# joaobuibergen/roms-trunk-mgh

Hardware: AMD Instinct MI355X
Metric: simulated-days/wall-sec (higher is better)
Workload: dtype f64; 1 GPU; BENCHMARK3 2048x256x30 NT=2 nonlinear 3-D step incl. 59 step2d calls, U3/C4 tracer advection, analytic atmospheric forcing, bulk fluxes + KPP + diagnostics every step; tiling=1x1, halo_transport=none, rccl_ranks=0, graph_exchanges=1, ndtfast=20, finite=True

## Files before the change

roms_trunk_mgh_amd/csrc/advect.h:

```cpp
#pragma once
#include <type_traits>
#include "roms_dev.h"

template <int HADV>
__device__ __forceinline__ double hflux(double Hflx, double tm1, double t0, double dm1, double d0, double dp1)
{
  if constexpr (HADV == ADV_C2) {
    return Hflx * 0.5 * (tm1 + t0);
  } else if constexpr (HADV == ADV_MPDATA) {
    const double cff1 = fmax(Hflx, 0.0), cff2 = fmin(Hflx, 0.0);
    return cff1 * tm1 + cff2 * t0;
  } else if constexpr (HADV == ADV_U3) {
    const double curv_m1 = d0 - dm1;
    const double curv_0 = dp1 - d0;
    const double cff1 = 1.0 / 6.0;
    return Hflx * 0.5 * (tm1 + t0) -
           cff1 * (curv_m1 * fmax(Hflx, 0.0) + curv_0 * fmin(Hflx, 0.0));
  } else if constexpr (HADV == ADV_A4) {
    const double eps = 1.0E-16;
    double g_m1, g_0;
    double cff = 2.0 * d0 * dm1;
    g_m1 = (cff > eps) ? cff / (d0 + dm1) : 0.0;
    cff = 2.0 * dp1 * d0;
    g_0 = (cff > eps) ? cff / (dp1 + d0) : 0.0;
// ... 147 lines not shown
  f.FEjp1 = hflux<HADV>(s.hv1, tk, s.yp1, dy0, dyp1, dyp2);
  return f;
}
template <int VADV>
__device__ __forceinline__ double vflux_level(int k, int N, double Wk, double tkm1, double tk, double tkp1, double tkp2,
                                              const double *spl, const double *a4cf)
{
  if (k == N) return 0.0;
  if constexpr (VADV == ADV_SPLINES) return spl[k];
  else {
    double cfk = 0.0, cfk1 = 0.0;
    if constexpr (VADV == ADV_A4) { cfk = a4cf[k]; cfk1 = a4cf[k + 1]; }
    return vflux<VADV>(k, N, Wk, tkm1, tk, tkp1, tkp2, cfk, cfk1);
  }
}
__device__ __forceinline__ void thomas_row(double dt, double hz_m1, double ohz_m1, double hz, double ohz, double akt_m2,
                                           double akt_m1, double akt_0, double t_m1, double t_0, double CFm, double DCm,
                                           double &CF, double &DC)
{
  const double cff6 = 1.0 / 6.0, cff3r = 1.0 / 3.0;
  const double fc = cff6 * hz_m1 - dt * akt_m2 * ohz_m1;
  const double cf = cff6 * hz - dt * akt_0 * ohz;
  const double bc = cff3r * (hz_m1 + hz) + dt * akt_m1 * (ohz_m1 + ohz);
  const double cff = 1.0 / (bc - fc * CFm);
  CF = cff * cf;
  DC = cff * (t_0 - t_m1 - fc * DCm);
}

static inline int adv_pair(int ha, int va)
{
// ... 25 lines not shown
```

roms_trunk_mgh_amd/csrc/k_mix.hip:

```cpp
#include "roms_dev.h"

int roms_entry_check(const char *name);

namespace {

__device__ __forceinline__ double dmin0(double a) { return a < 0.0 ? a : 0.0; }
__device__ __forceinline__ double dmax0(double a) { return a > 0.0 ? a : 0.0; }

template <bool STAB>
__device__ __forceinline__ double tdiff(double a, double b, double a2, double b2)
{
  if constexpr (STAB) return 0.75 * (a - b) + 0.25 * (a2 - b2);
  else return a - b;
}

struct Lap4 {
  double *lap;
  int i0, i1, j0, j1;
  int closed[4];
  int itrc;
  int nstp;
};

template <int MODE>
__device__ __forceinline__ void lap4_store(const roms_bounds_t &b, const Lap4 &L, long ni, int i, int j, long a, double val)
{
  const gd_t lap = (gd_t)L.lap;
  lap[a] = val;
  if (!b.EWperiodic) {
    if (b.west_edge && i == b.Istr) lap[a - 1] = L.closed[LBS_WEST] ? 0.0 : val;
    if (b.east_edge && i == b.Iend) lap[a + 1] = L.closed[LBS_EAST] ? 0.0 : val;
  }
  if (!b.NSperiodic) {
    if (b.south_edge && j == b.Jstr) lap[a - ni] = L.closed[LBS_SOUTH] ? 0.0 : val;
    if (b.north_edge && j == b.Jend) lap[a + ni] = L.closed[LBS_NORTH] ? 0.0 : val;
  }
}

template <int MODE, bool ISO, bool STAB = false>
__global__ void __launch_bounds__(BLK_X *BLK_Y)
k_t3dmix_geo(const RomsDev *__restrict__ c, int nrhs, int nnew, Lap4 L)
{
  DEV_PROLOGUE(c)
  const int ilo = MODE == 1 ? L.i0 : b.Istr, ihi = MODE == 1 ? L.i1 : b.Iend;
  const int jlo = MODE == 1 ? L.j0 : b.Jstr, jhi = MODE == 1 ? L.j1 : b.Jend;
  const TileTr tt = decode_tile_tracer(ihi - ilo + 1, jhi - jlo + 1, MODE == 0 ? b.NT : 1);
  if (!tt.valid) return;
  const int i = ilo + tt.bx * BLK_X + threadIdx.x;
  const int j = jlo + tt.by * BLK_Y + threadIdx.y;
  const int itrc = MODE == 0 ? 1 + tt.itr : L.itrc;
  if (i > ihi || j > jhi) return;
  const double dt = c->p.dt;
  const double *__restrict__ T = MODE == 2 ? L.lap : c->F.t + ((long)(nrhs - 1) + 3L * (itrc - 1)) * n3r;
  static_assert(!(STAB && MODE == 2), "the second biharmonic operator acts on LapT alone");
  const double *__restrict__ S = STAB ? c->F.t + ((long)(L.nstp - 1) + 3L * (itrc - 1)) * n3r : T;
  double *__restrict__ tn = c->F.t + ((long)(nnew - 1) + 3L * (itrc - 1)) * n3r;
  const double *__restrict__ z_r = ISO ? c->F.pden : c->F.z_r;
// ... 16 lines not shown
    mx0 = mx0 * umaskw(c, c0); mx1 = mx1 * umaskw(c, c0 + 1);
    my0 = my0 * vmaskw(c, c0); my1 = my1 * vmaskw(c, c0 + ni);
  }
  const double cfx0 = 0.25 * (d2[c0] + d2[c0 - 1]) * c->F.on_u[c0];
  const double cfx1 = 0.25 * (d2[c0 + 1] + d2[c0]) * c->F.on_u[c0 + 1];
  const double cfe0 = 0.25 * (d2[c0] + d2[c0 - ni]) * c->F.om_v[c0];
  const double cfe1 = 0.25 * (d2[c0 + ni] + d2[c0]) * c->F.om_v[c0 + ni];
  const double cfs = 0.5 * d2[c0];
  const double cdt = dt * pm[c0] * pn[c0];
  double zx0_a, zx1_a, tx0_a, tx1_a, ze0_a, ze1_a, te0_a, te1_a;
  double zx0_b, zx1_b, tx0_b, tx1_b, ze0_b, ze1_b, te0_b, te1_b;
  double dzm_a = 0.0, dz0_a = 0.0, dzp_a = 0.0, dzs_a = 0.0, dzn_a = 0.0;
  double dzm_b, dz0_b, dzp_b, dzs_b, dzn_b;
  double FS_a = 0.0, FS_b;
  double fsf_b = 0.0;
  struct LvIn { double Tm1, T01, Tp1, Ts1, Tn1, Zm1, Z01, Zp1, Zs1, Zn1, hz0, hzm, hzp, hzs, hzn, tn, zz1;
                double Sm1, S01, Sp1, Ss1, Sn1;
                double zzm1, zzp1, zzs1, zzn1; };
  const gcd_t gT = (gcd_t)T, gS = (gcd_t)S, gZ = (gcd_t)z_r, gHz = (gcd_t)Hz;
  const gd_t gtn = (gd_t)tn;
  auto load_level = [&](int k) {
    LvIn L;
    const long ck = c0 + (long)(k - 1) * nij;
    const long cu = (k < N) ? ck + nij : ck;
    L.Tm1 = gT[cu - 1]; L.T01 = gT[cu]; L.Tp1 = gT[cu + 1]; L.Ts1 = gT[cu - ni]; L.Tn1 = gT[cu + ni];
    if constexpr (STAB) { L.Sm1 = gS[cu - 1]; L.S01 = gS[cu]; L.Sp1 = gS[cu + 1]; L.Ss1 = gS[cu - ni]; L.Sn1 = gS[cu + ni]; }
    else L.Sm1 = L.S01 = L.Sp1 = L.Ss1 = L.Sn1 = 0.0;
    L.Zm1 = gZ[cu - 1]; L.Z01 = gZ[cu]; L.Zp1 = gZ[cu + 1]; L.Zs1 = gZ[cu - ni]; L.Zn1 = gZ[cu + ni];
    L.hz0 = gHz[ck]; L.hzm = gHz[ck - 1]; L.hzp = gHz[ck + 1]; L.hzs = gHz[ck - ni]; L.hzn = gHz[ck + ni];
    L.tn = gtn[ck];
    if constexpr (ISO) L.zz1 = ((gcd_t)zz)[cu]; else L.zz1 = 0.0;
    L.zzm1 = L.zzp1 = L.zzs1 = L.zzn1 = 0.0;
    if (minstrat) {
      const gcd_t gz = (gcd_t)zz;
      L.zzm1 = gz[cu - 1]; L.zzp1 = gz[cu + 1]; L.zzs1 = gz[cu - ni]; L.zzn1 = gz[cu + ni];
    }
    return L;
  };
  double Tm = T[c0 - 1], T0 = T[c0], Tp = T[c0 + 1], Ts = T[c0 - ni], Tn = T[c0 + ni];
  double Sm = 0.0, S0 = 0.0, Sp = 0.0, Ss = 0.0, Sn = 0.0;
  if constexpr (STAB) { Sm = S[c0 - 1]; S0 = S[c0]; Sp = S[c0 + 1]; Ss = S[c0 - ni]; Sn = S[c0 + ni]; }
  double Zm = z_r[c0 - 1], Z0 = z_r[c0], Zp = z_r[c0 + 1], Zs = z_r[c0 - ni], Zn = z_r[c0 + ni];
  double zzc = ISO ? zz[c0] : 0.0;
  double zzm = 0.0, zzp = 0.0, zzs = 0.0, zzn = 0.0;
  if (minstrat) { zzm = zz[c0 - 1]; zzp = zz[c0 + 1]; zzs = zz[c0 - ni]; zzn = zz[c0 + ni]; }
  zx0_b = mx0 * (Z0 - Zm); tx0_b = mx0 * tdiff<STAB>(T0, Tm, S0, Sm);
  zx1_b = mx1 * (Zp - Z0); tx1_b = mx1 * tdiff<STAB>(Tp, T0, Sp, S0);
  ze0_b = my0 * (Z0 - Zs); te0_b = my0 * tdiff<STAB>(T0, Ts, S0, Ss);
  ze1_b = my1 * (Zn - Z0); te1_b = my1 * tdiff<STAB>(Tn, T0, Sn, S0);
  LvIn cur = load_level(1);
  for (int k = 1; k <= N; k++) {
    const long ck = c0 + (long)(k - 1) * nij;
    LvIn nxt = cur;
    if (k < N) nxt = load_level(k + 1);
    zx0_a = zx0_b; zx1_a = zx1_b; tx0_a = tx0_b; tx1_a = tx1_b;
    ze0_a = ze0_b; ze1_a = ze1_b; te0_a = te0_b; te1_a = te1_b;
    if (k < N) {
      const double Tm1 = cur.Tm1, T01 = cur.T01, Tp1 = cur.Tp1, Ts1 = cur.Ts1, Tn1 = cur.Tn1;
      const double Zm1 = cur.Zm1, Z01 = cur.Z01, Zp1 = cur.Zp1, Zs1 = cur.Zs1, Zn1 = cur.Zn1;
      const double Sm1 = cur.Sm1, S01 = cur.S01, Sp1 = cur.Sp1, Ss1 = cur.Ss1, Sn1 = cur.Sn1;
      zx0_b = mx0 * (Z01 - Zm1); tx0_b = mx0 * tdiff<STAB>(T01, Tm1, S01, Sm1);
      zx1_b = mx1 * (Zp1 - Z01); tx1_b = mx1 * tdiff<STAB>(Tp1, T01, Sp1, S01);
      ze0_b = my0 * (Z01 - Zs1); te0_b = my0 * tdiff<STAB>(T01, Ts1, S01, Ss1);
      ze1_b = my1 * (Zn1 - Z01); te1_b = my1 * tdiff<STAB>(Tn1, T01, Sn1, S01);
      { const double q = vscale(Zm, Zm1, cur.zzm1 - zzm); dzm_b = q * tdiff<STAB>(Tm1, Tm, Sm1, Sm); }
      { const double q = vscale(Z0, Z01, cur.zz1 - zzc); dz0_b = q * tdiff<STAB>(T01, T0, S01, S0);
        if constexpr (ISO) { fsf_b = q * (cur.zz1 - zzc); zzc = cur.zz1; } }
// ... 37 lines not shown
        c1 = f1(ze0_a); c2 = f1(ze1_b); c3 = f2(ze0_b); c4 = f2(ze1_a);
        cff = cff + cfs * (c1 * (c1 * dz0_b - te0_a) + c2 * (c2 * dz0_b - te1_b) +
                           c3 * (c3 * dz0_b - te0_b) + c4 * (c4 * dz0_b - te1_a));
        FS_b = cff * fsf_b;
      }
    } else FS_b = 0.0;
    if constexpr (MODE == 1) {
      const double cff = pm[c0] * pn[c0];
      const double cff1 = 1.0 / hz0;
      lap4_store<MODE>(b, L, ni, i, j, ck, cff1 * (cff * (FX1 - FX0 + FE1 - FE0) + (FS_b - FS_a)));
    } else {
      const double cff1 = cdt * (FX1 - FX0);
      const double cff2 = cdt * (FE1 - FE0);
      const double cff3 = dt * (FS_b - FS_a);
      const double cff4 = cff1 + cff2 + cff3;
      if constexpr (MODE == 0) gtn[ck] = cur.tn + cff4;
      else gtn[ck] = cur.tn - cff4;
    }
    cur = nxt;
    dzm_a = dzm_b; dz0_a = dz0_b; dzp_a = dzp_b; dzs_a = dzs_b; dzn_a = dzn_b;
    FS_a = FS_b;
  }
}

template <bool STAB, bool DIA = false>
__global__ void __launch_bounds__(BLK_X *BLK_Y)
k_t3dmix2_s(const RomsDev *__restrict__ c, int nrhs, int nnew, int nstp)
{
  DEV_PROLOGUE(c)
  const TileTr tt = decode_tile_tracer(b.Iend - b.Istr + 1, b.Jend - b.Jstr + 1, b.NT);
  if (!tt.valid) return;
// ... 80 lines not shown
    double FE1 = cfe1 * (Hz[ck + ni] + h0) * tdiff<STAB>(T[ck + ni], t0, sn, s0);
    if constexpr (MODE == 1) {
      const double cff = 1.0 / h0;
      lap4_store<MODE>(b, L, ni, i, j, ck, pmn * cff * (FX1 - FX0 + FE1 - FE0));
    } else {
      if (masking) { FX0 = FX0 * um0; FX1 = FX1 * um1; FE0 = FE0 * vm0; FE1 = FE1 * vm1; }
      const double cff1 = cdt * (FX1 - FX0);
      const double cff2 = cdt * (FE1 - FE0);
      tn[ck] = tn[ck] - (cff1 + cff2);
    }
  }
}

}

static int t3dmix2_launch(const roms_step_idx_t *s)
{
  const roms_bounds_t &b = g_ctx.b;
  const dim3 grid = grid_tile_tracer(b.Iend - b.Istr + 1, b.Jend - b.Jstr + 1, b.NT);
  const bool stab = g_ctx.p.ts_mix_stability != 0;
  Lap4 L{};
  L.nstp = s->nstp;
  if (g_ctx.p.mix_iso_ts) {
    if (stab) hipLaunchKernelGGL((k_t3dmix_geo<0, true, true>), grid, block2d(), 0, g_ctx.stream, g_ctx.devc, s->nrhs, s->nnew, L);
    else hipLaunchKernelGGL((k_t3dmix_geo<0, true>), grid, block2d(), 0, g_ctx.stream, g_ctx.devc, s->nrhs, s->nnew, L);
  } else if (g_ctx.p.mix_geo_ts) {
    if (stab) hipLaunchKernelGGL((k_t3dmix_geo<0, false, true>), grid, block2d(), 0, g_ctx.stream, g_ctx.devc, s->nrhs, s->nnew, L);
    else hipLaunchKernelGGL((k_t3dmix_geo<0, false>), grid, block2d(), 0, g_ctx.stream, g_ctx.devc, s->nrhs, s->nnew, L);
  } else if (g_ctx.p.mix_s_ts && dia_on()) {
    if (stab) hipLaunchKernelGGL((k_t3dmix2_s<true, true>), grid, block2d(), 0, g_ctx.stream, g_ctx.devc, s->nrhs, s->nnew, s->nstp);
    else hipLaunchKernelGGL((k_t3dmix2_s<false, true>), grid, block2d(), 0, g_ctx.stream, g_ctx.devc, s->nrhs, s->nnew, s->nstp);
  } else if (g_ctx.p.mix_s_ts) {
    if (stab) hipLaunchKernelGGL(k_t3dmix2_s<true>, grid, block2d(), 0, g_ctx.stream, g_ctx.devc, s->nrhs, s->nnew, s->nstp);
    else hipLaunchKernelGGL(k_t3dmix2_s<false>, grid, block2d(), 0, g_ctx.stream, g_ctx.devc, s->nrhs, s->nnew, s->nstp);
  } else
    return roms_fail("roms_hip_t3dmix2", "no tracer mixing option (MIX_ISO_TS / MIX_GEO_TS / MIX_S_TS) selected");
  KERNEL_CHECK("k_t3dmix2");
  return 0;
}

extern "C" int roms_hip_t3dmix2(const roms_step_idx_t *s)
{
  int rc = roms_entry_check("roms_hip_t3dmix2");
  if (rc) return rc;
  if ((rc = dia_check("roms_hip_t3dmix2"))) return rc;
  if (dia_on() && !g_ctx.p.ts_dif2)
    return roms_fail("roms_hip_t3dmix2", "diagnostics: ts_dif2 is off, the iT?dif terms have no planes (NDT = 6)");
  ScopedTimer tm("t3dmix2");
  return t3dmix2_launch(s);
}

extern "C" int roms_hip_t3dmix4(const roms_step_idx_t *s)
{
  int rc = roms_entry_check("roms_hip_t3dmix4");
  if (rc) return rc;
  const roms_bounds_t &b = g_ctx.b;
  const roms_params_t &p = g_ctx.p;
  if (!p.ts_dif4) return roms_fail("roms_hip_t3dmix4", "TS_DIF4 is not set (roms_params_t.ts_dif4)");
  if ((rc = dia_check("roms_hip_t3dmix4"))) return rc;
  if (!p.mix_iso_ts && !p.mix_geo_ts && !p.mix_s_ts)
    return roms_fail("roms_hip_t3dmix4", "no tracer mixing option (MIX_ISO_TS / MIX_GEO_TS / MIX_S_TS) selected");
  ScopedTimer tm("t3dmix4");
  const bool stab = p.ts_mix_stability != 0;
  Lap4 L;
  L.lap = g_ctx.hostc.ws3[1];
// ... 28 lines not shown
```

roms_trunk_mgh_amd/csrc/k_pre_step3d.hip:

```cpp
#include "roms_dev.h"
#include "advect.h"

int roms_entry_check(const char *name);

namespace {

template <int HADV, int VADV, int NMAX, bool MASK, bool DIA = false>
__global__ void __launch_bounds__(BLK_X *BLK_Y)
k_pre_t(const RomsDev *__restrict__ c, int nstp, int nnew, int first_step, int itrc0, int ntr)
{
  DEV_PROLOGUE(c)
  const TileCol tc = tile_column(b, itrc0, ntr);
  if (!tc.valid) return;
  const int i = tc.i, j = tc.j, itrc = tc.itrc;
  const roms_params_t &p = c->p;
  const double dt = p.dt;
  const gcd_t ts = (gcd_t)tracer_level(c, nstp, itrc, n3r);
  const gd_t t3 = (gd_t)tracer_level(c, 3, itrc, n3r);
  const gd_t tn = (gd_t)tracer_level(c, nnew, itrc, n3r);
  const ColFields f = column_fields(c);
  const gcd_t z_r = (gcd_t)(c->F.z_r);
  const gcd_t z_w = (gcd_t)(c->F.z_w);
  const gcd_t Akt = tracer_akt(c, itrc, n3w);
  const long c0 = I2(i, j);
  const Walls wl = column_walls(c, i, j);
  const double Gamma = (HADV == ADV_MPDATA) ? 0.5 : 1.0 / 6.0;
  const double GammaV = (VADV == ADV_MPDATA) ? 0.5 : 1.0 / 6.0;
  double cff, cff1, cff2;
  if (first_step) { cff = 0.5 * dt; cff1 = 1.0; cff2 = 0.0; }
  else { cff = (1.0 - Gamma) * dt; cff1 = 0.5 + Gamma; cff2 = 0.5 - Gamma; }
  const double cpp = cff * GF(pm)[c0] * GF(pn)[c0];
  const double cppv = (first_step ? 0.5 * dt : (1.0 - GammaV) * dt) * GF(pm)[c0] * GF(pn)[c0];
  const double cff3 = dt * (1.0 - p.lambda);
  const bool nonlocal = p.lmd_nonlocal && itrc <= b.NAT;
  const bool solar = p.solar_source && itrc == 1;
  const gcd_t ghats = (gcd_t)(c->F.ghats + (long)((itrc <= b.NAT ? itrc : 1) - 1) * n3w);
  const gcd_t AktN = (gcd_t)(c->F.Akt + (long)((itrc <= b.NAT ? itrc : 1) - 1) * n3w);
  const double srf = GF(srflx)[c0];
  const double dsrf = c->p.wet_dry ? (dt * srf) * GF(rmask_wet)[c0] : dt * srf;
  const double zwN = z_w[c0 + (long)N * nij];
  const double fac1 = -1.0 / p.swfrac_mu1, fac2 = -1.0 / p.swfrac_mu2, fac3 = p.swfrac_r1;

  double a4cf[(VADV == ADV_A4) ? NMAX + 2 : 1];
  double spl[(VADV == ADV_SPLINES) ? NMAX + 1 : 1];
  if constexpr (VADV == ADV_A4) a4_slopes<NMAX>(ts, c0, nij, N, a4cf);
  if constexpr (VADV == ADV_SPLINES) spline_w<true, NMAX>(ts, f.Hz, f.W, c0, nij, N, spl);

  const bool src_cell = c->src.n > 0 && src_cell_any(c, c0, ni);
  double tkm1 = 0.0, tk = ts[c0], tkp1 = (N >= 2) ? ts[c0 + nij] : 0.0, tkp2;
  double FCprev = 0.0;
  double FDprev = dt * GF(btflx)[c0 + (long)(itrc - 1) * nij];
  double w_km1 = f.W[c0];
  double zr_k = (cff3 != 0.0) ? z_r[c0] : 0.0;
  for (int k = 1; k <= N; k++) {
    const long ck = c0 + (long)(k - 1) * nij;
    tkp2 = (k + 2 <= N) ? ts[ck + 2 * nij] : 0.0;
    HStencil s;
    s.xm1 = ts[ck - 1]; s.xp1 = ts[ck + 1];
    s.xm2 = wl.w ? 0.0 : ts[ck - 2];
    s.xp2 = wl.e ? 0.0 : ts[ck + 2];
    s.ym1 = ts[ck - ni]; s.yp1 = ts[ck + ni];
    s.ym2 = wl.s ? 0.0 : ts[ck - 2 * ni];
    s.yp2 = wl.n ? 0.0 : ts[ck + 2 * ni];
    s.hu0 = f.Huon[ck]; s.hu1 = f.Huon[ck + 1];
    s.hv0 = f.Hvom[ck]; s.hv1 = f.Hvom[ck + ni];
    Faces fx = cell_faces<HADV, MASK>(tk, s, wl, c, c0, ni);
    if (src_cell)
      src_cell_fluxes<true>(c, c0, ck, ni, k, itrc, nullptr, fx.FXi, fx.FXip1, fx.FEj, fx.FEjp1);
    const double hz = f.Hz[ck];
    const double tnn = tn[ck];
    double t3v = hz * (cff1 * tk + cff2 * tnn) - cpp * (fx.FXip1 - fx.FXi + fx.FEjp1 - fx.FEj);
    const double w_k = f.W[ck + nij];
    const double FCk = vflux_level<VADV>(k, N, w_k, tkm1, tk, tkp1, tkp2, spl, a4cf);
    const double DCk = 1.0 / (hz - cppv * (s.hu1 - s.hu0 + s.hv1 - s.hv0 + (w_k - w_km1)));
    t3v = DCk * (t3v - cppv * (FCk - FCprev));
    t3[ck] = t3v;
    double FDk;
    if (k == N) FDk = dt * GF(stflx)[c0 + (long)(itrc - 1) * nij];
    else {
      if (cff3 != 0.0) {
        const double zr_k1 = z_r[ck + nij];
        const double cz = 1.0 / (zr_k1 - zr_k);
        FDk = cff3 * cz * Akt[ck + nij] * (tkp1 - tk);
        zr_k = zr_k1;
      } else {
        FDk = 0.0;
      }
      if (nonlocal) FDk = FDk - dt * AktN[ck + nij] * ghats[ck + nij];
      if (solar) {
        const double Z = zwN - z_w[ck + nij];
        const double swdk = exp(Z * fac1) * fac3 + exp(Z * fac2) * (1.0 - fac3);
        FDk = FDk + dsrf * swdk;
      }
    }
    const double hzt = hz * tk, dFD = FDk - FDprev;
    tn[ck] = hzt + dFD;
    if constexpr (DIA) {
      DIA_PLANE(c, DIA_iTrate, itrc, n3r)[ck] = hzt;
      DIA_PLANE(c, DIA_iTvdif, itrc, n3r)[ck] = dFD;
    }
    FDprev = FDk;
    FCprev = FCk;
    w_km1 = w_k;
    tkm1 = tk; tk = tkp1; tkp1 = tkp2;
  }
}

__global__ void __launch_bounds__(BLK_X *BLK_Y)
k_pre_uv(const RomsDev *__restrict__ c, int nstp, int nnew, int nrhs, int stage)
{
  DEV_PROLOGUE(c)
  const Blk XB = xcd_block();
  const int i = b.Istr + XB.x * BLK_X + threadIdx.x;
  const int j = b.Jstr + XB.y * BLK_Y + threadIdx.y;
  if (i > b.Iend || j > b.Jend) return;
  const roms_params_t &p = c->p;
  const double dt = p.dt;
  const double cff3 = dt * (1.0 - p.lambda);
  const gcd_t z_r = (gcd_t)(c->F.z_r);
// ... 42 lines not shown
      } else if (stage == 1) {
        const double a = vk * 0.5 * hzs;
        const double c3 = 0.5 * DC0;
        out = a - c3 * r2[ck + nij] + d;
      } else {
        const double a = vk * 0.5 * hzs;
        out = a + DC0 * ((5.0 / 12.0) * r1[ck + nij] - (16.0 / 12.0) * r2[ck + nij]) + d;
      }
      vnew[ck] = out;
      FCprev = FCk;
      vk = vk1;
    }
  }
}

template <int HADV, int VADV>
int launch_pre_t(const roms_step_idx_t *s, int itrc0, int ntr)
{
  typedef void (*PreKernel)(const RomsDev *, int, int, int, int, int);
  const roms_bounds_t &b = g_ctx.b;
  const dim3 grid = grid_tile_tracer(b.Iend - b.Istr + 1, b.Jend - b.Jstr + 1, ntr);
  const int first = s->iic == s->ntfirst;
  if (b.N > ROMS_MAXN) return roms_fail("roms_hip_pre_step3d", "N > 64 not instantiated");
  PreKernel kernel = kernel_for_n(b.N, [](auto nm) -> PreKernel { return k_pre_t<HADV, VADV, nm.value, false>; });
  if constexpr (HADV != ADV_MPDATA)
    if (g_ctx.p.masking)
      kernel = kernel_for_n(b.N, [](auto nm) -> PreKernel { return k_pre_t<HADV, VADV, nm.value, true>; });
  if constexpr (HADV != ADV_MPDATA && VADV != ADV_MPDATA)
    if (dia_on())
      kernel = g_ctx.p.masking ? k_pre_t<HADV, VADV, ROMS_MAXN, true, true> : k_pre_t<HADV, VADV, ROMS_MAXN, false, true>;
  hipLaunchKernelGGL(kernel, grid, block2d(), 0, g_ctx.stream, g_ctx.devc, s->nstp, s->nnew, first, itrc0, ntr);
  KERNEL_CHECK("k_pre_t");
  return 0;
}

}

static int pre_step3d_tracers(const roms_step_idx_t *s)
{
  const roms_bounds_t &b = g_ctx.b;
  const roms_params_t &p = g_ctx.p;
  int rc = 0;
  {
    int it = 1;
    while (it <= b.NT) {
      const int n = adv_run_length(p, b.NT, it);
      switch (adv_pair(p.Hadv[it - 1], p.Vadv[it - 1])) {
      case ADV_U3 * 16 + ADV_C4:   rc = launch_pre_t<ADV_U3, ADV_C4>(s, it, n); break;
      case ADV_A4 * 16 + ADV_A4:   rc = launch_pre_t<ADV_A4, ADV_A4>(s, it, n); break;
      case ADV_C4 * 16 + ADV_C4:   rc = launch_pre_t<ADV_C4, ADV_C4>(s, it, n); break;
      case ADV_C2 * 16 + ADV_C2:   rc = launch_pre_t<ADV_C2, ADV_C2>(s, it, n); break;
      case ADV_U3 * 16 + ADV_SPLINES: rc = launch_pre_t<ADV_U3, ADV_SPLINES>(s, it, n); break;
      case ADV_C4 * 16 + ADV_SPLINES: rc = launch_pre_t<ADV_C4, ADV_SPLINES>(s, it, n); break;
      case ADV_A4 * 16 + ADV_SPLINES: rc = launch_pre_t<ADV_A4, ADV_SPLINES>(s, it, n); break;
      case ADV_MPDATA * 16 + ADV_MPDATA: rc = launch_pre_t<ADV_MPDATA, ADV_MPDATA>(s, it, n); break;
      case ADV_HSIMT * 16 + ADV_HSIMT: rc = launch_pre_t<ADV_MPDATA, ADV_MPDATA>(s, it, n); break;
      case ADV_U3 * 16 + ADV_HSIMT: rc = launch_pre_t<ADV_U3, ADV_MPDATA>(s, it, n); break;
      case ADV_C4 * 16 + ADV_HSIMT: rc = launch_pre_t<ADV_C4, ADV_MPDATA>(s, it, n); break;
      case ADV_A4 * 16 + ADV_HSIMT: rc = launch_pre_t<ADV_A4, ADV_MPDATA>(s, it, n); break;
      case ADV_C2 * 16 + ADV_HSIMT: rc = launch_pre_t<ADV_C2, ADV_MPDATA>(s, it, n); break;
      default:
        return roms_fail("roms_hip_pre_step3d", "advection scheme pair not implemented (MPDATA and HSIMT only as H+V pairs)");
      }
      if (rc) return rc;
      it += n;
    }
  }
  const long n3r = (long)(b.UBi - b.LBi + 1) * (b.UBj - b.LBj + 1) * b.N;
  for (int it = 1; it <= b.NT; it++)
    if ((rc = bc_t3d(3, it, s->nstp))) return rc;
  halo_batch_begin();
  for (int it = 1; it <= b.NT; it++) halo_exchange3d(GT_R, b.N, g_ctx.dev[FID_t] + (2L + 3L * (it - 1)) * n3r);
  return halo_batch_end();
}

static int pre_step3d_uv(const roms_step_idx_t *s)
{
  const roms_bounds_t &b = g_ctx.b;
  const int stage = (s->iic == s->ntfirst) ? 0 : (s->iic == s->ntfirst + 1 ? 1 : 2);
  hipLaunchKernelGGL(k_pre_uv, grid2d(b.Iend - b.Istr + 1, b.Jend - b.Jstr + 1), block2d(), 0, g_ctx.stream,
                     g_ctx.devc, s->nstp, s->nnew, s->nrhs, stage);
  KERNEL_CHECK("k_pre_uv");
  return 0;
}

extern "C" int roms_hip_pre_step3d(const roms_step_idx_t *s)
{
  int rc = roms_entry_check("roms_hip_pre_step3d");
  if (rc) return rc;
  if ((rc = check_lbc())) return rc;
  if (g_ctx.b.N < 4) return roms_fail("roms_hip_pre_step3d", "needs N >= 4 levels (the vertical stencils of the column read k-1 .. k+2)");
  if ((rc = dia_check("roms_hip_pre_step3d"))) return rc;
  ScopedTimer tm("pre_step3d");
  if ((rc = pre_step3d_uv(s))) return rc;
  return pre_step3d_tracers(s);
}
```

roms_trunk_mgh_amd/csrc/k_rhs3d.hip:

```cpp
#include "roms_dev.h"

namespace {

#define Gadv (-0.25)

struct T3 {
  const double *u, *v, *Hu, *Hv, *Hz;
  int i0, j0;
  int Istr, Iend, Jstr, Jend;
  bool s_edge, n_edge, w_edge, e_edge;
  __device__ __forceinline__ int at(int i, int j) const { return (i - i0) + (j - j0) * TP; }
};

__device__ __forceinline__ int ex_uxx(const T3 &L, int i) {
  if (L.w_edge && i == L.Istr) return L.Istr + 1;
  if (L.e_edge && i == L.Iend + 1) return L.Iend;
  return i;
}
__device__ __forceinline__ int ey_uee(const T3 &L, int j) {
  if (L.s_edge && j == L.Jstr - 1) return L.Jstr;
  if (L.n_edge && j == L.Jend + 1) return L.Jend;
  return j;
}
__device__ __forceinline__ int ex_vxx(const T3 &L, int i) {
// ... 391 lines not shown
                                            : (spl ? k_rhs3d_lds<ROMS_UVH_U3, ROMS_UVV_SPLINES> : k_rhs3d_lds<ROMS_UVH_U3, ROMS_UVV_C4W>);
  hipLaunchKernelGGL(kernel, grid2d(b.Iend - b.Istr + 1, b.Jend - b.Jstr + 1), block2d(), 0, g_ctx.stream,
                     g_ctx.devc, s->nrhs);
  KERNEL_CHECK("k_rhs3d_lds");
  if (spl) {
    const dim3 grid((unsigned)((b.Iend - b.Istr + BLK_X) / BLK_X), (unsigned)(b.Jend - b.Jstr + 1), 1), block(BLK_X, 1, 1);
    if (b.N <= 16) hipLaunchKernelGGL(k_rhs3d_vspline<16>, grid, block, 0, g_ctx.stream, g_ctx.devc, s->nrhs);
    else if (b.N <= 32) hipLaunchKernelGGL(k_rhs3d_vspline<32>, grid, block, 0, g_ctx.stream, g_ctx.devc, s->nrhs);
    else if (b.N <= 48) hipLaunchKernelGGL(k_rhs3d_vspline<48>, grid, block, 0, g_ctx.stream, g_ctx.devc, s->nrhs);
    else hipLaunchKernelGGL(k_rhs3d_vspline<64>, grid, block, 0, g_ctx.stream, g_ctx.devc, s->nrhs);
    KERNEL_CHECK("k_rhs3d_vspline");
  }
  return 0;
}

extern "C" int roms_hip_rhs3d(const roms_step_idx_t *s)
{
  int rc = roms_entry_check("roms_hip_rhs3d");
  if (rc) return rc;
  if ((rc = roms_uv_adv_check("roms_hip_rhs3d"))) return rc;
  if ((rc = roms_hip_pre_step3d(s))) return rc;
  if ((rc = roms_hip_prsgrd(s))) return rc;
  if (g_ctx.p.ts_dif2 && (rc = roms_hip_t3dmix2(s))) return rc;
  if (g_ctx.p.ts_dif4 && (rc = roms_hip_t3dmix4(s))) return rc;
  if ((rc = roms_hip_rhs3d_tile(s))) return rc;
  if (g_ctx.p.uv_vis2 && (rc = roms_hip_uv3dmix2(s))) return rc;
  if (g_ctx.p.uv_vis4 && (rc = roms_hip_uv3dmix4(s))) return rc;
  return 0;
}
```

roms_trunk_mgh_amd/csrc/roms_dev.h:

```cpp
#pragma once
#include <hip/hip_runtime.h>
#include <cstdio>
#include <cstring>
#include <string>
#include "roms_hip.h"

#define ROMS_NWS3 10

struct RomsSrc {
  int n;
  int ltr[ROMS_MAXNT];
  const int *I, *J, *D;
  const double *Qbar;
  const double *Qsrc;
  const double *Tsrc;
  const int *umap, *vmap;
  const int *wmap;
  const int *cells;
  int ncell;
  double *save;
};

struct RomsClima {
  int m2, m3, nt;
// ... 295 lines not shown
int dia_arrays(const char *name[4], const double *base[4], long count[4]);
int bc_zeta(int kout, const roms_step_idx_t *s);
int bc_u2d(int kout, const roms_step_idx_t *s);
int bc_v2d(int kout, const roms_step_idx_t *s);
int bc_u3d(int nout, int nstp);
int bc_v3d(int nout, int nstp);
int bc_t3d(int nout, int itrc, int nstp);
bool lbc2d_all_closed();
int lbc_code(const roms_params_t &p, int sd, int v);
int bc_w3d(double *A);
int bc_generic(int gtype_var, int lbv, double *A, int nk);
void snapshot_release();
void snapshot_forget(int field_id);
void diag_release();
int check_lbc();
int roms_rowm_prepare();
void roms_rowm_invalidate();
bool roms_rowm_is_table_field(int id);
void roms_rowm_release();
void step2d_graphs_release();
```

Baseline: 0.2365 simulated-days/s.

## Defer tracer t(nnew) start into t3dmix2 and pair tracers in pre_step3d

When harmonic geopotential or isopycnal tracer mixing runs with lambda=1, no stability mixing and no diagnostics, pre_step3d no longer writes t(nnew). It writes only t(3). The Hz*t plus vertical-flux start of t(nnew) is computed inside the t3dmix2 kernel, which already writes that plane, so one read-modify-write pass over t(nnew) is removed. The deferred pre_t kernel also processes two tracers per thread, sharing the Huon, Hvom, Hz and W loads and the DCk divide. In exchange it uses more registers and adds template instantiations, and it only applies under restrictive runtime conditions.

```diff
diff --git a/roms_trunk_mgh_amd/csrc/advect.h b/roms_trunk_mgh_amd/csrc/advect.h
--- a/roms_trunk_mgh_amd/csrc/advect.h
+++ b/roms_trunk_mgh_amd/csrc/advect.h
@@ -185,6 +185,68 @@
     return vflux<VADV>(k, N, Wk, tkm1, tk, tkp1, tkp2, cfk, cfk1);
   }
 }
+struct VStart {
+  double dt, cff3, dsrf, zwN, fac1, fac2, fac3;
+  bool nonlocal, solar;
+  gcd_t Akt, AktN, ghats, z_r, z_w;
+  int itrc;
+};
+__device__ __forceinline__ VStart vstart_column(const RomsDev *__restrict__ c, int itrc, long c0, long nij, long n3w)
+{
+  const roms_params_t &p = c->p;
+  const roms_bounds_t &b = c->b;
+  VStart v;
+  v.dt = p.dt;
+  v.cff3 = p.dt * (1.0 - p.lambda);
+  v.nonlocal = p.lmd_nonlocal && itrc <= b.NAT;
+  v.solar = p.solar_source && itrc == 1;
+  v.Akt = tracer_akt(c, itrc, n3w);
+  v.ghats = (gcd_t)(c->F.ghats + (long)((itrc <= b.NAT ? itrc : 1) - 1) * n3w);
+  v.AktN = (gcd_t)(c->F.Akt + (long)((itrc <= b.NAT ? itrc : 1) - 1) * n3w);
+  v.z_r = (gcd_t)(c->F.z_r);
+  v.z_w = (gcd_t)(c->F.z_w);
+  const double srf = GF(srflx)[c0];
+  v.dsrf = p.wet_dry ? (p.dt * srf) * GF(rmask_wet)[c0] : p.dt * srf;
+  v.zwN = v.z_w[c0 + (long)b.N * nij];
+  v.fac1 = -1.0 / p.swfrac_mu1; v.fac2 = -1.0 / p.swfrac_mu2; v.fac3 = p.swfrac_r1;
+  v.itrc = itrc;
+  return v;
+}
+struct VStartIn { double akn, gh, zwk; };
+__device__ __forceinline__ VStartIn vstart_load(const VStart &v, long cku)
+{
+  VStartIn r{0.0, 0.0, 0.0};
+  if (v.nonlocal) { r.akn = v.AktN[cku]; r.gh = v.ghats[cku]; }
+  if (v.solar) r.zwk = v.z_w[cku];
+  return r;
+}
+__device__ __forceinline__ double vstart_bottom(const RomsDev *__restrict__ c, const VStart &v, long c0, long nij)
+{
+  return v.dt * GF(btflx)[c0 + (long)(v.itrc - 1) * nij];
+}
+template <bool EXPL>
+__device__ __forceinline__ double vstart_flux(const RomsDev *__restrict__ c, const VStart &v, int k, int N, long c0, long nij,
+                                              long cku, const VStartIn &in, double tk, double tkp1, double &zr_k)
+{
+  if (k == N) return v.dt * GF(stflx)[c0 + (long)(v.itrc - 1) * nij];
+  double FDk = 0.0;
+  if constexpr (EXPL) {
+    if (v.cff3 != 0.0) {
+      const double zr_k1 = v.z_r[cku];
+      const double cz = 1.0 / (zr_k1 - zr_k);
+      FDk = v.cff3 * cz * v.Akt[cku] * (tkp1 - tk);
+      zr_k = zr_k1;
+    }
+  }
+  if (v.nonlocal) FDk = FDk - v.dt * in.akn * in.gh;
+  if (v.solar) {
+    const double Z = v.zwN - in.zwk;
+    const double swdk = exp(Z * v.fac1) * v.fac3 + exp(Z * v.fac2) * (1.0 - v.fac3);
+    FDk = FDk + v.dsrf * swdk;
+  }
+  return FDk;
+}
+
 __device__ __forceinline__ void thomas_row(double dt, double hz_m1, double ohz_m1, double hz, double ohz, double akt_m2,
                                            double akt_m1, double akt_0, double t_m1, double t_0, double CFm, double DCm,
                                            double &CF, double &DC)
diff --git a/roms_trunk_mgh_amd/csrc/k_mix.hip b/roms_trunk_mgh_amd/csrc/k_mix.hip
--- a/roms_trunk_mgh_amd/csrc/k_mix.hip
+++ b/roms_trunk_mgh_amd/csrc/k_mix.hip
@@ -1,4 +1,5 @@
 #include "roms_dev.h"
+#include "advect.h"
 
 int roms_entry_check(const char *name);
 
@@ -37,10 +38,11 @@
   }
 }
 
-template <int MODE, bool ISO, bool STAB = false>
+template <int MODE, bool ISO, bool STAB = false, bool START = false>
 __global__ void __launch_bounds__(BLK_X *BLK_Y)
 k_t3dmix_geo(const RomsDev *__restrict__ c, int nrhs, int nnew, Lap4 L)
 {
+  static_assert(!START || (MODE == 0 && !STAB), "the corrector's start goes with t3dmix2 alone");
   DEV_PROLOGUE(c)
   const int ilo = MODE == 1 ? L.i0 : b.Istr, ihi = MODE == 1 ? L.i1 : b.Iend;
   const int jlo = MODE == 1 ? L.j0 : b.Jstr, jhi = MODE == 1 ? L.j1 : b.Jend;
@@ -87,9 +89,13 @@
   double dzm_b, dz0_b, dzp_b, dzs_b, dzn_b;
   double FS_a = 0.0, FS_b;
   double fsf_b = 0.0;
+  VStart vs{};
+  double FDprev = 0.0, zr_unused = 0.0;
+  if constexpr (START) { vs = vstart_column(c, itrc, c0, nij, n3w); FDprev = vstart_bottom(c, vs, c0, nij); }
   struct LvIn { double Tm1, T01, Tp1, Ts1, Tn1, Zm1, Z01, Zp1, Zs1, Zn1, hz0, hzm, hzp, hzs, hzn, tn, zz1;
                 double Sm1, S01, Sp1, Ss1, Sn1;
-                double zzm1, zzp1, zzs1, zzn1; };
+                double zzm1, zzp1, zzs1, zzn1;
+                double akn, gh, zwk; };
   const gcd_t gT = (gcd_t)T, gS = (gcd_t)S, gZ = (gcd_t)z_r, gHz = (gcd_t)Hz;
   const gd_t gtn = (gd_t)tn;
   auto load_level = [&](int k) {
@@ -101,7 +107,10 @@
     else L.Sm1 = L.S01 = L.Sp1 = L.Ss1 = L.Sn1 = 0.0;
     L.Zm1 = gZ[cu - 1]; L.Z01 = gZ[cu]; L.Zp1 = gZ[cu + 1]; L.Zs1 = gZ[cu - ni]; L.Zn1 = gZ[cu + ni];
     L.hz0 = gHz[ck]; L.hzm = gHz[ck - 1]; L.hzp = gHz[ck + 1]; L.hzs = gHz[ck - ni]; L.hzn = gHz[ck + ni];
-    L.tn = gtn[ck];
+    if constexpr (START) L.tn = 0.0; else L.tn = gtn[ck];
+    L.akn = L.gh = L.zwk = 0.0;
+    if constexpr (START)
+      if (k < N) { const VStartIn in = vstart_load(vs, ck + nij); L.akn = in.akn; L.gh = in.gh; L.zwk = in.zwk; }
     if constexpr (ISO) L.zz1 = ((gcd_t)zz)[cu]; else L.zz1 = 0.0;
     L.zzm1 = L.zzp1 = L.zzs1 = L.zzn1 = 0.0;
     if (minstrat) {
@@ -124,6 +133,7 @@
   LvIn cur = load_level(1);
   for (int k = 1; k <= N; k++) {
     const long ck = c0 + (long)(k - 1) * nij;
+    const double Tk = T0;
     LvIn nxt = cur;
     if (k < N) nxt = load_level(k + 1);
     zx0_a = zx0_b; zx1_a = zx1_b; tx0_a = tx0_b; tx1_a = tx1_b;
@@ -191,7 +201,13 @@
       const double cff2 = cdt * (FE1 - FE0);
       const double cff3 = dt * (FS_b - FS_a);
       const double cff4 = cff1 + cff2 + cff3;
-      if constexpr (MODE == 0) gtn[ck] = cur.tn + cff4;
+      if constexpr (START) {
+        const VStartIn in{cur.akn, cur.gh, cur.zwk};
+        const double FDk = vstart_flux<false>(c, vs, k, N, c0, nij, ck + nij, in, Tk, 0.0, zr_unused);
+        const double hzt = hz0 * Tk, dFD = FDk - FDprev;
+        gtn[ck] = (hzt + dFD) + cff4;
+        FDprev = FDk;
+      } else if constexpr (MODE == 0) gtn[ck] = cur.tn + cff4;
       else gtn[ck] = cur.tn - cff4;
     }
     cur = nxt;
@@ -302,14 +318,19 @@
 
 }
 
-static int t3dmix2_launch(const roms_step_idx_t *s)
+static int t3dmix2_launch(const roms_step_idx_t *s, bool fused)
 {
   const roms_bounds_t &b = g_ctx.b;
   const dim3 grid = grid_tile_tracer(b.Iend - b.Istr + 1, b.Jend - b.Jstr + 1, b.NT);
   const bool stab = g_ctx.p.ts_mix_stability != 0;
   Lap4 L{};
   L.nstp = s->nstp;
-  if (g_ctx.p.mix_iso_ts) {
+  if (fused) {
+    if (stab || dia_on() || !(g_ctx.p.mix_iso_ts || g_ctx.p.mix_geo_ts))
+      return roms_fail("roms_hip_t3dmix2", "internal: the fused start of t(nnew) was asked for where it is not built");
+    if (g_ctx.p.mix_iso_ts) hipLaunchKernelGGL((k_t3dmix_geo<0, true, false, true>), grid, block2d(), 0, g_ctx.stream, g_ctx.devc, s->nrhs, s->nnew, L);
+    else hipLaunchKernelGGL((k_t3dmix_geo<0, false, false, true>), grid, block2d(), 0, g_ctx.stream, g_ctx.devc, s->nrhs, s->nnew, L);
+  } else if (g_ctx.p.mix_iso_ts) {
     if (stab) hipLaunchKernelGGL((k_t3dmix_geo<0, true, true>), grid, block2d(), 0, g_ctx.stream, g_ctx.devc, s->nrhs, s->nnew, L);
     else hipLaunchKernelGGL((k_t3dmix_geo<0, true>), grid, block2d(), 0, g_ctx.stream, g_ctx.devc, s->nrhs, s->nnew, L);
   } else if (g_ctx.p.mix_geo_ts) {
@@ -327,7 +348,7 @@
   return 0;
 }
 
-extern "C" int roms_hip_t3dmix2(const roms_step_idx_t *s)
+int t3dmix2_entry(const roms_step_idx_t *s, bool fused)
 {
   int rc = roms_entry_check("roms_hip_t3dmix2");
   if (rc) return rc;
@@ -335,8 +356,10 @@
   if (dia_on() && !g_ctx.p.ts_dif2)
     return roms_fail("roms_hip_t3dmix2", "diagnostics: ts_dif2 is off, the iT?dif terms have no planes (NDT = 6)");
   ScopedTimer tm("t3dmix2");
-  return t3dmix2_launch(s);
-}
+  return t3dmix2_launch(s, fused);
+}
+
+extern "C" int roms_hip_t3dmix2(const roms_step_idx_t *s) { return t3dmix2_entry(s, false); }
 
 extern "C" int roms_hip_t3dmix4(const roms_step_idx_t *s)
 {
diff --git a/roms_trunk_mgh_amd/csrc/k_pre_step3d.hip b/roms_trunk_mgh_amd/csrc/k_pre_step3d.hip
--- a/roms_trunk_mgh_amd/csrc/k_pre_step3d.hip
+++ b/roms_trunk_mgh_amd/csrc/k_pre_step3d.hip
@@ -5,23 +5,20 @@
 
 namespace {
 
-template <int HADV, int VADV, int NMAX, bool MASK, bool DIA = false>
+template <int HADV, int VADV, int NMAX, bool MASK, bool DIA = false, bool DEFER = false, int NTR = 1>
 __global__ void __launch_bounds__(BLK_X *BLK_Y)
 k_pre_t(const RomsDev *__restrict__ c, int nstp, int nnew, int first_step, int itrc0, int ntr)
 {
+  static_assert(NTR == 1 || (VADV != ADV_A4 && VADV != ADV_SPLINES && !DIA), "pairs: no whole-column arrays, no diagnostics");
+  static_assert(!(DIA && DEFER), "diagnostics keep the two kernels");
   DEV_PROLOGUE(c)
   const TileCol tc = tile_column(b, itrc0, ntr);
   if (!tc.valid) return;
-  const int i = tc.i, j = tc.j, itrc = tc.itrc;
+  const int i = tc.i, j = tc.j;
+  const int itrc1 = itrc0 + NTR * (tc.itrc - itrc0);
   const roms_params_t &p = c->p;
   const double dt = p.dt;
-  const gcd_t ts = (gcd_t)tracer_level(c, nstp, itrc, n3r);
-  const gd_t t3 = (gd_t)tracer_level(c, 3, itrc, n3r);
-  const gd_t tn = (gd_t)tracer_level(c, nnew, itrc, n3r);
   const ColFields f = column_fields(c);
-  const gcd_t z_r = (gcd_t)(c->F.z_r);
-  const gcd_t z_w = (gcd_t)(c->F.z_w);
-  const gcd_t Akt = tracer_akt(c, itrc, n3w);
   const long c0 = I2(i, j);
   const Walls wl = column_walls(c, i, j);
   const double Gamma = (HADV == ADV_MPDATA) ? 0.5 : 1.0 / 6.0;
@@ -31,78 +28,81 @@
   else { cff = (1.0 - Gamma) * dt; cff1 = 0.5 + Gamma; cff2 = 0.5 - Gamma; }
   const double cpp = cff * GF(pm)[c0] * GF(pn)[c0];
   const double cppv = (first_step ? 0.5 * dt : (1.0 - GammaV) * dt) * GF(pm)[c0] * GF(pn)[c0];
-  const double cff3 = dt * (1.0 - p.lambda);
-  const bool nonlocal = p.lmd_nonlocal && itrc <= b.NAT;
-  const bool solar = p.solar_source && itrc == 1;
-  const gcd_t ghats = (gcd_t)(c->F.ghats + (long)((itrc <= b.NAT ? itrc : 1) - 1) * n3w);
-  const gcd_t AktN = (gcd_t)(c->F.Akt + (long)((itrc <= b.NAT ? itrc : 1) - 1) * n3w);
-  const double srf = GF(srflx)[c0];
-  const double dsrf = c->p.wet_dry ? (dt * srf) * GF(rmask_wet)[c0] : dt * srf;
-  const double zwN = z_w[c0 + (long)N * nij];
-  const double fac1 = -1.0 / p.swfrac_mu1, fac2 = -1.0 / p.swfrac_mu2, fac3 = p.swfrac_r1;
-
+
+  gcd_t ts[NTR];
+  gd_t t3[NTR], tn[NTR];
+  VStart vs[NTR];
+  double zr_k[NTR], FDprev[NTR];
+  double tkm1[NTR], tk[NTR], tkp1[NTR], tkp2[NTR];
+  double FCprev[NTR];
   double a4cf[(VADV == ADV_A4) ? NMAX + 2 : 1];
   double spl[(VADV == ADV_SPLINES) ? NMAX + 1 : 1];
-  if constexpr (VADV == ADV_A4) a4_slopes<NMAX>(ts, c0, nij, N, a4cf);
-  if constexpr (VADV == ADV_SPLINES) spline_w<true, NMAX>(ts, f.Hz, f.W, c0, nij, N, spl);
+#pragma unroll
+  for (int q = 0; q < NTR; q++) {
+    ts[q] = (gcd_t)tracer_level(c, nstp, itrc1 + q, n3r);
+    t3[q] = (gd_t)tracer_level(c, 3, itrc1 + q, n3r);
+    tn[q] = (gd_t)tracer_level(c, nnew, itrc1 + q, n3r);
+    if constexpr (!DEFER) {
+      vs[q] = vstart_column(c, itrc1 + q, c0, nij, n3w);
+      FDprev[q] = vstart_bottom(c, vs[q], c0, nij);
+      zr_k[q] = (vs[q].cff3 != 0.0) ? vs[q].z_r[c0] : 0.0;
+    }
+    tkm1[q] = 0.0; tk[q] = ts[q][c0]; tkp1[q] = (N >= 2) ? ts[q][c0 + nij] : 0.0;
+    FCprev[q] = 0.0;
+  }
+  if constexpr (VADV == ADV_A4) a4_slopes<NMAX>(ts[0], c0, nij, N, a4cf);
+  if constexpr (VADV == ADV_SPLINES) spline_w<true, NMAX>(ts[0], f.Hz, f.W, c0, nij, N, spl);
 
   const bool src_cell = c->src.n > 0 && src_cell_any(c, c0, ni);
-  double tkm1 = 0.0, tk = ts[c0], tkp1 = (N >= 2) ? ts[c0 + nij] : 0.0, tkp2;
-  double FCprev = 0.0;
-  double FDprev = dt * GF(btflx)[c0 + (long)(itrc - 1) * nij];
   double w_km1 = f.W[c0];
-  double zr_k = (cff3 != 0.0) ? z_r[c0] : 0.0;
   for (int k = 1; k <= N; k++) {
     const long ck = c0 + (long)(k - 1) * nij;
-    tkp2 = (k + 2 <= N) ? ts[ck + 2 * nij] : 0.0;
-    HStencil s;
-    s.xm1 = ts[ck - 1]; s.xp1 = ts[ck + 1];
-    s.xm2 = wl.w ? 0.0 : ts[ck - 2];
-    s.xp2 = wl.e ? 0.0 : ts[ck + 2];
-    s.ym1 = ts[ck - ni]; s.yp1 = ts[ck + ni];
-    s.ym2 = wl.s ? 0.0 : ts[ck - 2 * ni];
-    s.yp2 = wl.n ? 0.0 : ts[ck + 2 * ni];
-    s.hu0 = f.Huon[ck]; s.hu1 = f.Huon[ck + 1];
-    s.hv0 = f.Hvom[ck]; s.hv1 = f.Hvom[ck + ni];
-    Faces fx = cell_faces<HADV, MASK>(tk, s, wl, c, c0, ni);
-    if (src_cell)
-      src_cell_fluxes<true>(c, c0, ck, ni, k, itrc, nullptr, fx.FXi, fx.FXip1, fx.FEj, fx.FEjp1);
-    const double hz = f.Hz[ck];
-    const double tnn = tn[ck];
-    double t3v = hz * (cff1 * tk + cff2 * tnn) - cpp * (fx.FXip1 - fx.FXi + fx.FEjp1 - fx.FEj);
-    const double w_k = f.W[ck + nij];
-    const double FCk = vflux_level<VADV>(k, N, w_k, tkm1, tk, tkp1, tkp2, spl, a4cf);
-    const double DCk = 1.0 / (hz - cppv * (s.hu1 - s.hu0 + s.hv1 - s.hv0 + (w_k - w_km1)));
-    t3v = DCk * (t3v - cppv * (FCk - FCprev));
-    t3[ck] = t3v;
-    double FDk;
-    if (k == N) FDk = dt * GF(stflx)[c0 + (long)(itrc - 1) * nij];
-    else {
-      if (cff3 != 0.0) {
-        const double zr_k1 = z_r[ck + nij];
-        const double cz = 1.0 / (zr_k1 - zr_k);
-        FDk = cff3 * cz * Akt[ck + nij] * (tkp1 - tk);
-        zr_k = zr_k1;
-      } else {
-        FDk = 0.0;
-      }
-      if (nonlocal) FDk = FDk - dt * AktN[ck + nij] * ghats[ck + nij];
-      if (solar) {
-        const double Z = zwN - z_w[ck + nij];
-        const double swdk = exp(Z * fac1) * fac3 + exp(Z * fac2) * (1.0 - fac3);
-        FDk = FDk + dsrf * swdk;
-      }
-    }
-    const double hzt = hz * tk, dFD = FDk - FDprev;
-    tn[ck] = hzt + dFD;
-    if constexpr (DIA) {
-      DIA_PLANE(c, DIA_iTrate, itrc, n3r)[ck] = hzt;
-      DIA_PLANE(c, DIA_iTvdif, itrc, n3r)[ck] = dFD;
-    }
-    FDprev = FDk;
-    FCprev = FCk;
+    HStencil s[NTR];
+    double tnn[NTR];
+#pragma unroll
+    for (int q = 0; q < NTR; q++) {
+      const gcd_t t = ts[q];
+      tkp2[q] = (k + 2 <= N) ? t[ck + 2 * nij] : 0.0;
+      s[q].xm1 = t[ck - 1]; s[q].xp1 = t[ck + 1];
+      s[q].xm2 = wl.w ? 0.0 : t[ck - 2];
+      s[q].xp2 = wl.e ? 0.0 : t[ck + 2];
+      s[q].ym1 = t[ck - ni]; s[q].yp1 = t[ck + ni];
+      s[q].ym2 = wl.s ? 0.0 : t[ck - 2 * ni];
+      s[q].yp2 = wl.n ? 0.0 : t[ck + 2 * ni];
+      if constexpr (NTR > 1) tnn[q] = tn[q][ck];
+    }
+    const double hu0 = f.Huon[ck], hu1 = f.Huon[ck + 1], hv0 = f.Hvom[ck], hv1 = f.Hvom[ck + ni];
+    double hz, w_k, DCk;
+#pragma unroll
+    for (int q = 0; q < NTR; q++) {
+      const int itrc = itrc1 + q;
+      s[q].hu0 = hu0; s[q].hu1 = hu1; s[q].hv0 = hv0; s[q].hv1 = hv1;
+      Faces fx = cell_faces<HADV, MASK>(tk[q], s[q], wl, c, c0, ni);
+      if (src_cell)
+        src_cell_fluxes<true>(c, c0, ck, ni, k, itrc, nullptr, fx.FXi, fx.FXip1, fx.FEj, fx.FEjp1);
+      if (q == 0) hz = f.Hz[ck];
+      if constexpr (NTR == 1) tnn[q] = tn[q][ck];
+      double t3v = hz * (cff1 * tk[q] + cff2 * tnn[q]) - cpp * (fx.FXip1 - fx.FXi + fx.FEjp1 - fx.FEj);
+      if (q == 0) w_k = f.W[ck + nij];
+      const double FCk = vflux_level<VADV>(k, N, w_k, tkm1[q], tk[q], tkp1[q], tkp2[q], spl, a4cf);
+      if (q == 0) DCk = 1.0 / (hz - cppv * (hu1 - hu0 + hv1 - hv0 + (w_k - w_km1)));
+      t3v = DCk * (t3v - cppv * (FCk - FCprev[q]));
+      t3[q][ck] = t3v;
+      if constexpr (!DEFER) {
+        const VStartIn in = (k < N) ? vstart_load(vs[q], ck + nij) : VStartIn{0.0, 0.0, 0.0};
+        const double FDk = vstart_flux<true>(c, vs[q], k, N, c0, nij, ck + nij, in, tk[q], tkp1[q], zr_k[q]);
+        const double hzt = hz * tk[q], dFD = FDk - FDprev[q];
+        tn[q][ck] = hzt + dFD;
+        if constexpr (DIA) {
+          DIA_PLANE(c, DIA_iTrate, itrc, n3r)[ck] = hzt;
+          DIA_PLANE(c, DIA_iTvdif, itrc, n3r)[ck] = dFD;
+        }
+        FDprev[q] = FDk;
+      }
+      FCprev[q] = FCk;
+      tkm1[q] = tk[q]; tk[q] = tkp1[q]; tkp1[q] = tkp2[q];
+    }
     w_km1 = w_k;
-    tkm1 = tk; tk = tkp1; tkp1 = tkp2;
   }
 }
 
@@ -175,29 +175,58 @@
   }
 }
 
-template <int HADV, int VADV>
-int launch_pre_t(const roms_step_idx_t *s, int itrc0, int ntr)
+template <int HADV, int VADV, bool DEFER, int NTR>
+int launch_pre_t_n(const roms_step_idx_t *s, int itrc0, int nthr)
 {
   typedef void (*PreKernel)(const RomsDev *, int, int, int, int, int);
   const roms_bounds_t &b = g_ctx.b;
-  const dim3 grid = grid_tile_tracer(b.Iend - b.Istr + 1, b.Jend - b.Jstr + 1, ntr);
+  const dim3 grid = grid_tile_tracer(b.Iend - b.Istr + 1, b.Jend - b.Jstr + 1, nthr);
   const int first = s->iic == s->ntfirst;
   if (b.N > ROMS_MAXN) return roms_fail("roms_hip_pre_step3d", "N > 64 not instantiated");
-  PreKernel kernel = kernel_for_n(b.N, [](auto nm) -> PreKernel { return k_pre_t<HADV, VADV, nm.value, false>; });
-  if constexpr (HADV != ADV_MPDATA)
-    if (g_ctx.p.masking)
-      kernel = kernel_for_n(b.N, [](auto nm) -> PreKernel { return k_pre_t<HADV, VADV, nm.value, true>; });
-  if constexpr (HADV != ADV_MPDATA && VADV != ADV_MPDATA)
-    if (dia_on())
-      kernel = g_ctx.p.masking ? k_pre_t<HADV, VADV, ROMS_MAXN, true, true> : k_pre_t<HADV, VADV, ROMS_MAXN, false, true>;
-  hipLaunchKernelGGL(kernel, grid, block2d(), 0, g_ctx.stream, g_ctx.devc, s->nstp, s->nnew, first, itrc0, ntr);
+  PreKernel kernel;
+  if constexpr (NTR == 2) {
+    kernel = k_pre_t<HADV, VADV, ROMS_MAXN, false, false, DEFER, 2>;
+    if constexpr (HADV != ADV_MPDATA)
+      if (g_ctx.p.masking) kernel = k_pre_t<HADV, VADV, ROMS_MAXN, true, false, DEFER, 2>;
+  } else {
+    kernel = kernel_for_n(b.N, [](auto nm) -> PreKernel { return k_pre_t<HADV, VADV, nm.value, false, false, DEFER>; });
+    if constexpr (HADV != ADV_MPDATA)
+      if (g_ctx.p.masking)
+        kernel = kernel_for_n(b.N, [](auto nm) -> PreKernel { return k_pre_t<HADV, VADV, nm.value, true, false, DEFER>; });
+    if constexpr (HADV != ADV_MPDATA && VADV != ADV_MPDATA && !DEFER)
+      if (dia_on())
+        kernel = g_ctx.p.masking ? k_pre_t<HADV, VADV, ROMS_MAXN, true, true> : k_pre_t<HADV, VADV, ROMS_MAXN, false, true>;
+  }
+  hipLaunchKernelGGL(kernel, grid, block2d(), 0, g_ctx.stream, g_ctx.devc, s->nstp, s->nnew, first, itrc0, nthr);
   KERNEL_CHECK("k_pre_t");
   return 0;
 }
 
-}
-
-static int pre_step3d_tracers(const roms_step_idx_t *s)
+constexpr bool pre_t_pairs(int ha, int va)
+{
+  return (ha == ADV_U3 && va == ADV_C4) || (ha == ADV_C4 && va == ADV_C4) || (ha == ADV_C2 && va == ADV_C2) ||
+         (ha == ADV_MPDATA && va == ADV_MPDATA);
+}
+
+template <int HADV, int VADV>
+int launch_pre_t(const roms_step_idx_t *s, int itrc0, int ntr, bool fused)
+{
+  int rc = 0;
+  if constexpr (pre_t_pairs(HADV, VADV))
+    if (fused && ntr >= 2) {
+      const int np = ntr / 2;
+      rc = launch_pre_t_n<HADV, VADV, true, 2>(s, itrc0, np);
+      if (rc) return rc;
+      itrc0 += 2 * np;
+      ntr -= 2 * np;
+    }
+  if (ntr == 0) return 0;
+  return fused ? launch_pre_t_n<HADV, VADV, true, 1>(s, itrc0, ntr) : launch_pre_t_n<HADV, VADV, false, 1>(s, itrc0, ntr);
+}
+
+}
+
+static int pre_step3d_tracers(const roms_step_idx_t *s, bool fused)
 {
   const roms_bounds_t &b = g_ctx.b;
   const roms_params_t &p = g_ctx.p;
@@ -207,19 +236,19 @@
     while (it <= b.NT) {
       const int n = adv_run_length(p, b.NT, it);
       switch (adv_pair(p.Hadv[it - 1], p.Vadv[it - 1])) {
-      case ADV_U3 * 16 + ADV_C4:   rc = launch_pre_t<ADV_U3, ADV_C4>(s, it, n); break;
-      case ADV_A4 * 16 + ADV_A4:   rc = launch_pre_t<ADV_A4, ADV_A4>(s, it, n); break;
-      case ADV_C4 * 16 + ADV_C4:   rc = launch_pre_t<ADV_C4, ADV_C4>(s, it, n); break;
-      case ADV_C2 * 16 + ADV_C2:   rc = launch_pre_t<ADV_C2, ADV_C2>(s, it, n); break;
-      case ADV_U3 * 16 + ADV_SPLINES: rc = launch_pre_t<ADV_U3, ADV_SPLINES>(s, it, n); break;
-      case ADV_C4 * 16 + ADV_SPLINES: rc = launch_pre_t<ADV_C4, ADV_SPLINES>(s, it, n); break;
-      case ADV_A4 * 16 + ADV_SPLINES: rc = launch_pre_t<ADV_A4, ADV_SPLINES>(s, it, n); break;
-      case ADV_MPDATA * 16 + ADV_MPDATA: rc = launch_pre_t<ADV_MPDATA, ADV_MPDATA>(s, it, n); break;
-      case ADV_HSIMT * 16 + ADV_HSIMT: rc = launch_pre_t<ADV_MPDATA, ADV_MPDATA>(s, it, n); break;
-      case ADV_U3 * 16 + ADV_HSIMT: rc = launch_pre_t<ADV_U3, ADV_MPDATA>(s, it, n); break;
-      case ADV_C4 * 16 + ADV_HSIMT: rc = launch_pre_t<ADV_C4, ADV_MPDATA>(s, it, n); break;
-      case ADV_A4 * 16 + ADV_HSIMT: rc = launch_pre_t<ADV_A4, ADV_MPDATA>(s, it, n); break;
-      case ADV_C2 * 16 + ADV_HSIMT: rc = launch_pre_t<ADV_C2, ADV_MPDATA>(s, it, n); break;
+      case ADV_U3 * 16 + ADV_C4:   rc = launch_pre_t<ADV_U3, ADV_C4>(s, it, n, fused); break;
+      case ADV_A4 * 16 + ADV_A4:   rc = launch_pre_t<ADV_A4, ADV_A4>(s, it, n, fused); break;
+      case ADV_C4 * 16 + ADV_C4:   rc = launch_pre_t<ADV_C4, ADV_C4>(s, it, n, fused); break;
+      case ADV_C2 * 16 + ADV_C2:   rc = launch_pre_t<ADV_C2, ADV_C2>(s, it, n, fused); break;
+      case ADV_U3 * 16 + ADV_SPLINES: rc = launch_pre_t<ADV_U3, ADV_SPLINES>(s, it, n, fused); break;
+      case ADV_C4 * 16 + ADV_SPLINES: rc = launch_pre_t<ADV_C4, ADV_SPLINES>(s, it, n, fused); break;
+      case ADV_A4 * 16 + ADV_SPLINES: rc = launch_pre_t<ADV_A4, ADV_SPLINES>(s, it, n, fused); break;
+      case ADV_MPDATA * 16 + ADV_MPDATA: rc = launch_pre_t<ADV_MPDATA, ADV_MPDATA>(s, it, n, fused); break;
+      case ADV_HSIMT * 16 + ADV_HSIMT: rc = launch_pre_t<ADV_MPDATA, ADV_MPDATA>(s, it, n, fused); break;
+      case ADV_U3 * 16 + ADV_HSIMT: rc = launch_pre_t<ADV_U3, ADV_MPDATA>(s, it, n, fused); break;
+      case ADV_C4 * 16 + ADV_HSIMT: rc = launch_pre_t<ADV_C4, ADV_MPDATA>(s, it, n, fused); break;
+      case ADV_A4 * 16 + ADV_HSIMT: rc = launch_pre_t<ADV_A4, ADV_MPDATA>(s, it, n, fused); break;
+      case ADV_C2 * 16 + ADV_HSIMT: rc = launch_pre_t<ADV_C2, ADV_MPDATA>(s, it, n, fused); break;
       default:
         return roms_fail("roms_hip_pre_step3d", "advection scheme pair not implemented (MPDATA and HSIMT only as H+V pairs)");
       }
@@ -245,7 +274,7 @@
   return 0;
 }
 
-extern "C" int roms_hip_pre_step3d(const roms_step_idx_t *s)
+int pre_step3d_entry(const roms_step_idx_t *s, bool fused)
 {
   int rc = roms_entry_check("roms_hip_pre_step3d");
   if (rc) return rc;
@@ -254,5 +283,7 @@
   if ((rc = dia_check("roms_hip_pre_step3d"))) return rc;
   ScopedTimer tm("pre_step3d");
   if ((rc = pre_step3d_uv(s))) return rc;
-  return pre_step3d_tracers(s);
-}
+  return pre_step3d_tracers(s, fused);
+}
+
+extern "C" int roms_hip_pre_step3d(const roms_step_idx_t *s) { return pre_step3d_entry(s, false); }
diff --git a/roms_trunk_mgh_amd/csrc/k_rhs3d.hip b/roms_trunk_mgh_amd/csrc/k_rhs3d.hip
--- a/roms_trunk_mgh_amd/csrc/k_rhs3d.hip
+++ b/roms_trunk_mgh_amd/csrc/k_rhs3d.hip
@@ -429,14 +429,22 @@
   return 0;
 }
 
+static bool rhs3d_fuses_tstart(const roms_step_idx_t *s)
+{
+  const roms_params_t &p = g_ctx.p;
+  return p.ts_dif2 && (p.mix_geo_ts || p.mix_iso_ts) && !p.ts_mix_stability && p.lambda == 1.0 && !dia_on() &&
+         s->nrhs == s->nstp;
+}
+
 extern "C" int roms_hip_rhs3d(const roms_step_idx_t *s)
 {
   int rc = roms_entry_check("roms_hip_rhs3d");
   if (rc) return rc;
   if ((rc = roms_uv_adv_check("roms_hip_rhs3d"))) return rc;
-  if ((rc = roms_hip_pre_step3d(s))) return rc;
+  const bool fused = rhs3d_fuses_tstart(s);
+  if ((rc = pre_step3d_entry(s, fused))) return rc;
   if ((rc = roms_hip_prsgrd(s))) return rc;
-  if (g_ctx.p.ts_dif2 && (rc = roms_hip_t3dmix2(s))) return rc;
+  if (g_ctx.p.ts_dif2 && (rc = t3dmix2_entry(s, fused))) return rc;
   if (g_ctx.p.ts_dif4 && (rc = roms_hip_t3dmix4(s))) return rc;
   if ((rc = roms_hip_rhs3d_tile(s))) return rc;
   if (g_ctx.p.uv_vis2 && (rc = roms_hip_uv3dmix2(s))) return rc;
diff --git a/roms_trunk_mgh_amd/csrc/roms_dev.h b/roms_trunk_mgh_amd/csrc/roms_dev.h
--- a/roms_trunk_mgh_amd/csrc/roms_dev.h
+++ b/roms_trunk_mgh_amd/csrc/roms_dev.h
@@ -333,6 +333,8 @@
 void snapshot_forget(int field_id);
 void diag_release();
 int check_lbc();
+int pre_step3d_entry(const roms_step_idx_t *s, bool fused);
+int t3dmix2_entry(const roms_step_idx_t *s, bool fused);
 int roms_rowm_prepare();
 void roms_rowm_invalidate();
 bool roms_rowm_is_table_field(int id);
```

Result: faster. 0.2410 simulated-days/s (median of 6 runs) (+1.9%).
